# lucas-carmo/RAFT-testStuff

Hardware: AMD Instinct MI355X
Metric: sea-state cases/sec (converged RAO+PSD) (higher is better)
Workload: dtype f64; 1 GPU; C2: VolturnUS-S_example nw=1000, 512 JONSWAP sea states per GPU per step (step = per-heading wave tables + batched drag fixed point); nw=1000, submerged_nodes=53, nIter=4, headings=4, parallelism=case-sharded x1, clock_ramp_steps=920

## Files before the change

raft-teststuff_amd/csrc/rh_solve.hip:

```cpp
#include "rh_common.h"
#ifdef RH_VARIANTS
#include "../../tools/ubench/variants_src/rh_a0_common.h"
#endif

namespace rh {

#ifdef RH_PROF
static __device__ unsigned long long rh_prof[12];
#define PROF_T(v) const unsigned long long v = clock64()
#define PROF_ADD(i, x) if (tid == 0) atomicAdd(&rh_prof[i], (unsigned long long)(x))
#else
#define PROF_T(v)
#define PROF_ADD(i, x)
#endif

#ifdef RH_WGTIME
static __device__ unsigned long long rh_wgt[2 * 8192];
#endif

constexpr int kLT = 512;
constexpr int kLW = kLT / 64;
#ifndef RH_RING_A
#define RH_RING_A 4
#endif
#ifndef RH_RING_C
#define RH_RING_C 6
#endif
constexpr int kRingA1 = RH_RING_A;
constexpr int kRingC = RH_RING_C;
#ifndef RH_ONE_VOTE
#define RH_ONE_VOTE 0
#endif
#ifndef RH_OVERLAP
#define RH_OVERLAP 1
#endif
#ifndef RH_STATS_C
#define RH_STATS_C 1
#endif
#ifndef RH_XI_STORE
#define RH_XI_STORE 1
#endif
#define XI_STORE_MODE RH_XI_STORE
#ifndef RH_A_PAIR
#define RH_A_PAIR 1
#endif
constexpr int kAxC = 4;
#ifndef RH_JOINT_C
#define RH_JOINT_C 1
#endif
constexpr bool kJointC = RH_JOINT_C != 0;
#ifndef RH_JOINT_PARK
#define RH_JOINT_PARK 1
#endif
constexpr int kRingCJ = kRingC / 2;
static_assert(kRingC % 2 == 0, "the joint phase-C ring pairs its slots");
constexpr int kGhost = 1;
#ifndef RH_A_QUAD
#define RH_A_QUAD 1
#endif
#ifndef RH_LDS_LANE_BRANCH
#define RH_LDS_LANE_BRANCH 0
#endif

__device__ __forceinline__ int opaque_zero() {
  int z;
  asm volatile("s_mov_b32 %0, 0" : "=s"(z));
  return z;
}

__device__ __forceinline__ int lane_here() {
  int r;
  asm volatile("v_mbcnt_lo_u32_b32 %0, -1, 0\n\tv_mbcnt_hi_u32_b32 %0, -1, %0" : "=v"(r));
  return r;
}

template <int CTRL>
__device__ __forceinline__ double dpp_mov(double v) {
  const int lo = __builtin_amdgcn_mov_dpp(__double2loint(v), CTRL, 0xF, 0xF, true);
  const int hi = __builtin_amdgcn_mov_dpp(__double2hiint(v), CTRL, 0xF, 0xF, true);
  return __hiloint2double(hi, lo);
}

__device__ __forceinline__ double xsum32(double t) {
  const int lo = __double2loint(t), hi = __double2hiint(t);
  const auto a = __builtin_amdgcn_permlane32_swap(lo, lo, false, false);
  const auto b = __builtin_amdgcn_permlane32_swap(hi, hi, false, false);
  return __hiloint2double(b[0], a[0]) + __hiloint2double(b[1], a[1]);
}
__device__ __forceinline__ double xsum16(double t) {
  const int lo = __double2loint(t), hi = __double2hiint(t);
  const auto a = __builtin_amdgcn_permlane16_swap(lo, lo, false, false);
  const auto b = __builtin_amdgcn_permlane16_swap(hi, hi, false, false);
  return __hiloint2double(b[0], a[0]) + __hiloint2double(b[1], a[1]);
}

__device__ __forceinline__ double tbfly16(double (&u)[16], int lane) {
  const int i = lane & 15;
  const bool f0 = ((i ^ (i >> 2)) & 1) != 0, f1 = (((i >> 1) ^ (i >> 2)) & 1) != 0;
  const bool f2 = (((i >> 2) ^ (i >> 3)) & 1) != 0, f3 = ((i >> 3) & 1) != 0;
#pragma unroll
  for (int p = 0; p < 8; ++p) {
    const double keep = f0 ? u[p + 8] : u[p], send = f0 ? u[p] : u[p + 8];
    u[p] = keep + dpp_mov<0xB1>(send);
  }
#pragma unroll
  for (int p = 0; p < 4; ++p) {
    const double keep = f1 ? u[p + 4] : u[p], send = f1 ? u[p] : u[p + 4];
    u[p] = keep + dpp_mov<0x4E>(send);
  }
#pragma unroll
  for (int p = 0; p < 2; ++p) {
    const double keep = f2 ? u[p + 2] : u[p], send = f2 ? u[p] : u[p + 2];
    u[p] = keep + dpp_mov<0x141>(send);
  }
  {
    const double keep = f3 ? u[1] : u[0], send = f3 ? u[0] : u[1];
    u[0] = keep + dpp_mov<0x140>(send);
  }
  return xsum32(xsum16(u[0]));
}
__device__ __forceinline__ int tbfly16_index(int lane) {
  const int i = lane & 15;
  return 8 * ((i ^ (i >> 2)) & 1) + 4 * (((i >> 1) ^ (i >> 2)) & 1) + 2 * (((i >> 2) ^ (i >> 3)) & 1) + ((i >> 3) & 1);
}

__device__ __forceinline__ double tbfly3(double a, double b, double c, int lane) {
  const bool f0 = (lane & 1) != 0, f1 = (lane & 2) != 0;
  const double k0 = f0 ? c : a, s0 = f0 ? a : c;
  const double k1 = f0 ? 0.0 : b, s1 = f0 ? b : 0.0;
  const double u0 = k0 + dpp_mov<0xB1>(s0);
  const double u1 = k1 + dpp_mov<0xB1>(s1);
  double t = (f1 ? u1 : u0) + dpp_mov<0x4E>(f1 ? u0 : u1);
  t += dpp_mov<0x124>(t);
  t += dpp_mov<0x128>(t);
  return xsum32(xsum16(t));
}
__device__ __forceinline__ int tbfly3_index(int lane) { return 2 * (lane & 1) + ((lane >> 1) & 1); }

struct Bfly4 {
  bool f0, f1, f2;
  int vi;
  int vi8;
};
__device__ __forceinline__ Bfly4 bfly4_lane(int lane) {
  const int i = lane & 15;
  Bfly4 b;
  b.f0 = ((i ^ (i >> 2)) & 1) != 0;
  b.f1 = (((i >> 1) ^ (i >> 2)) & 1) != 0;
  b.f2 = (((i >> 2) ^ (i >> 3)) & 1) != 0;
  b.vi = lane >= 4 ? -1 : 2 * (lane & 1) + ((lane >> 1) & 1);
  b.vi8 = lane >= 8 ? -1 : 4 * b.f0 + 2 * b.f1 + b.f2;
  return b;
}
__device__ __forceinline__ double tbfly8(const double (&u)[8], const Bfly4& L) {
  const bool f0 = L.f0, f1 = L.f1, f2 = L.f2;
  double v[4], w[2];
#pragma unroll
  for (int p = 0; p < 4; ++p) v[p] = (f0 ? u[p + 4] : u[p]) + dpp_mov<0xB1>(f0 ? u[p] : u[p + 4]);
#pragma unroll
  for (int p = 0; p < 2; ++p) w[p] = (f1 ? v[p + 2] : v[p]) + dpp_mov<0x4E>(f1 ? v[p] : v[p + 2]);
  double t = (f2 ? w[1] : w[0]) + dpp_mov<0x141>(f2 ? w[0] : w[1]);
  t += dpp_mov<0x140>(t);
  return xsum32(xsum16(t));
}
__device__ __forceinline__ double tbfly4(double a, double b, double c, double d, const Bfly4& L) {
  const bool f0 = L.f0, f1 = L.f1;
  const double v0 = (f0 ? c : a) + dpp_mov<0xB1>(f0 ? a : c);
  const double v1 = (f0 ? d : b) + dpp_mov<0xB1>(f0 ? b : d);
  double t = (f1 ? v1 : v0) + dpp_mov<0x4E>(f1 ? v0 : v1);
  t += dpp_mov<0x141>(t);
  t += dpp_mov<0x140>(t);
  return xsum32(xsum16(t));
}

template <int CTRL, int ROWS>
__device__ __forceinline__ double dpp_mov_rows(double v) {
  const int lo = __builtin_amdgcn_update_dpp(0, __double2loint(v), CTRL, ROWS, 0xF, false);
  const int hi = __builtin_amdgcn_update_dpp(0, __double2hiint(v), CTRL, ROWS, 0xF, false);
  return __hiloint2double(hi, lo);
}

__device__ __forceinline__ double wave_sum63(double v) {
  v += dpp_mov<0xB1>(v);
  v += dpp_mov<0x4E>(v);
  v += dpp_mov<0x141>(v);
  v += dpp_mov<0x140>(v);
  v += dpp_mov_rows<0x142, 0xA>(v);
  v += dpp_mov_rows<0x143, 0xC>(v);
  return v;
}

__device__ __forceinline__ double t3to6_block(const double* Bm, double rx, double ry, double rz, int blk, int r, int c) {
  const double H[3][3] = {{0, rz, -ry}, {-rz, 0, rx}, {ry, -rx, 0}};
  double hc[3], hr[3];
#pragma unroll
  for (int k = 0; k < 3; ++k) {
    hc[k] = c == 0 ? H[k][0] : c == 1 ? H[k][1] : H[k][2];
    hr[k] = r == 0 ? H[0][k] : r == 1 ? H[1][k] : H[2][k];
  }
  double hcc[3];
#pragma unroll
  for (int k = 0; k < 3; ++k) hcc[k] = c == 0 ? H[0][k] : c == 1 ? H[1][k] : H[2][k];
  const double b0 = Bm[3 * r + c];
  const double b1 = Bm[3 * r + 0] * hc[0] + Bm[3 * r + 1] * hc[1] + Bm[3 * r + 2] * hc[2];
  double b2 = 0;
#pragma unroll
  for (int k = 0; k < 3; ++k) {
    const double HB = hr[0] * Bm[0 * 3 + k] + hr[1] * Bm[1 * 3 + k] + hr[2] * Bm[2 * 3 + k];
    b2 += HB * hcc[k];
  }
  return blk == 0 ? b0 : blk == 1 ? b1 : b2;
}

__host__ __device__ inline size_t solve_lds_smem(int nn, int nm, int NB, int LT = kLT, bool ser = false, int NP = 1) {
  const int LW = LT / 64;
  return sizeof(double) * ((size_t)(NP == 1 ? 12 * LT * NB : 0)
                           + (size_t)(ser && nn * 3 * LW < 27 ? 27 : nn * 3 * LW)
                           + (ser ? (size_t)0 : (size_t)nn * 36)
                           + (size_t)nn * 9
                           + (size_t)(nn + kGhost) * 6
                           + (size_t)(nn + kGhost)
                           + (size_t)nm * 18
                           + (size_t)2 * LT * NB * NP
                           + 36 + 108 + LW * 6 + 36
                           + LW)
         + sizeof(int) * ((size_t)nm + 6);
}

template <int NB, int LT = kLT, bool SER = false, int NP = 1>
__global__ __launch_bounds__(LT, LT >= 256 ? 512 / LT : 2) void k_solve_lds(CaseArgs a) {
  constexpr bool JC = kJointC && NB == 2 && LT == kLT && !SER && NP == 1;
  constexpr int LW = LT / 64;
  extern __shared__ __attribute__((aligned(16))) double smem[];
  const int tid = threadIdx.x, lane = tid & 63, wv = tid >> 6;
  const int wv_s = __builtin_amdgcn_readfirstlane(wv);
  PROF_T(tp0);
#ifdef RH_WGTIME
  const unsigned long long wgt0 = __builtin_amdgcn_s_memrealtime();
#endif
  const int slot = xcd_remap(blockIdx.x, a.c.ncase);
  const int ic = a.c.order ? a.c.order[slot] : slot;
#ifdef RH_VARIANTS
  const bool resume = a.resume != 0;
  const int stop_iter = a.stop_iter;
  if (resume && a.o.status[ic] != kCaseStopped) return;
#else
  constexpr bool resume = false;
  constexpr int stop_iter = 1 << 30;
#endif
  const rh_design& d = a.designs[a.c.design[ic]].d;
  const int nw = d.nw, nn = d.nn, nm = d.nm;
  const unsigned nw16 = (unsigned)nw * 16u;
  const double* __restrict__ node = d.node;
  const int head = a.c.head[ic];
  const size_t c6 = (size_t)ic * 6 * nw;
  const Buf bK = mkbuf(d.kproj + (size_t)head * nn * 3 * nw, (unsigned)nn * 3u * nw16);
  const Buf bFe = mkbuf(d.finer + (size_t)head * 6 * nw, 6u * nw16);
  const bool has_fx = a.c.fext != nullptr;
  const Buf bFx = mkbuf(has_fx ? a.c.fext + c6 : nullptr, has_fx ? 6u * nw16 : 0u);

  constexpr int NWP = LT * NB;
  constexpr int NBT = NB * NP;
  constexpr bool GX = NP > 1;
  constexpr int kRingA = GX ? 3 : kRingA1;
  constexpr bool kStatsC = RH_STATS_C && (XI_STORE_MODE == 1) && !SER && NB > 1;
#if RH_OVERLAP && !defined(RH_VARIANTS)
  constexpr bool kOv = !GX;
#else
  constexpr bool kOv = false;
#endif
  auto wave_maxes = [&](const double* m) {
    double mx = m[0];
    for (int w = 1; w < LW; ++w) mx = fmax(mx, m[w]);
    return mx;
  };
  cd* xl = reinterpret_cast<cd*>(smem);
  rh_c128* XL = a.o.Xi_last + c6;
  double* mbf = smem + (GX ? 0 : 12 * NWP);
  double* al = mbf + 18 * nm;
  double* red = al + 6 * (nn + kGhost);
  double* bm = red + (SER && nn * 3 * LW < 27 ? 27 : nn * 3 * LW);
  double* bd = bm + nn * 9;
  double* mbc = bd + 36;
  double* sred = mbc + 108;
  double* bsum = sred + LW * 6;
  double* bdn = bsum + 36;
  double* nt = bdn + (SER ? 0 : 36 * nn);
  double* lw = nt + nn + kGhost;
  double* lz = lw + NP * NWP;
  double* mred = lz + NP * NWP;
  int* mstart = reinterpret_cast<int*>(mred + LW);
  int* ax = reinterpret_cast<int*>(al);
  auto ax_node = [&](int k) { return k < nn ? __builtin_amdgcn_readfirstlane(ax[12 * k + 11]) : -1; };
  int* sflag = mstart + nm + 1;
  load_mbc(d, mbc, tid);
  for (int n = tid; n < nn; n += LT) {
    nt[n] = node[RH_NF_T * nn + n];
    const double aq = node[RH_NF_AQ * nn + n], cdq = node[RH_NF_CDQ * nn + n];
    const double ae = node[RH_NF_AEND * nn + n], cde = node[RH_NF_CDEND * nn + n];
    ax[12 * n + 10] = (a.all_axial || aq * cdq != 0.0 || ae * cde != 0.0) ? 1 : 0;
  }
  for (int e = tid; e < 18 * nm; e += LT) mbf[e] = d.memb[(e % 18) * nm + e / 18];
  for (int e = tid; e <= nm; e += LT) mstart[e] = e < nm ? d.mstart[e] : INT_MAX;
  for (int e = tid; e < 6 * kGhost; e += LT) al[6 * nn + e] = 0.0;
  for (int e = tid; e < kGhost; e += LT) nt[nn + e] = 0.0;
  if (tid < 5) sflag[tid] = 0;
  const int it0 = resume ? stop_iter : a.c.first_iter;
#ifdef RH_VARIANTS
  bool skip_a = a.a0 != 0 && it0 == 0;
#else
  constexpr bool skip_a = false;
#endif
  if (skip_a) {
#ifdef RH_VARIANTS
    const double* a0s = a0_block(a, ic, nw);
    const int nch = a0_chunks(nw);
    for (int e = tid; e < nn * 3; e += LT) {
      double s = 0;
      for (int ch = 0; ch < nch; ++ch) s += a0s[(size_t)ch * 3 * nn + e];
      red[e * LW] = s;
#pragma unroll
      for (int w = 1; w < LW; ++w) red[e * LW + w] = 0.0;
    }
    __syncthreads();
#endif
  }

  auto voff = [&](int b) { return (unsigned)(b < nw ? b : nw - 1) * 16u; };
  {
    const int spec = a.c.spectrum[ic];
    const double Hs = a.c.Hs[ic], Tp = a.c.Tp[ic], gam = a.c.gamma[ic];
    const rh_c128* XI0 = resume ? a.o.Xi_last + c6 : a.c.Xi_init ? a.c.Xi_init + c6 : nullptr;
#pragma unroll
    for (int j = 0; j < NBT; ++j) {
      const int b = tid + LT * j;
      const bool okb = b < nw;
      lw[b] = d.w[okb ? b : nw - 1];
#pragma unroll
      for (int c = 0; c < 6; ++c) {
        const cd x0 = okb ? (XI0 ? ld(XI0 + c * nw + b) : mk(a.c.XiStart, 0.0)) : mk(0.0, 0.0);
        if constexpr (GX) {
          if (okb && !resume) st(XL + c * nw + b, x0);
        } else {
          xl[c * NWP + b] = x0;
        }
      }
    }
#pragma unroll
    for (int j = 0; j < NBT; ++j) {
      const int b = tid + LT * j;
      const bool okb = b < nw;
      const double zz = sea_amplitude(spec, Hs, Tp, gam, lw[b], d.dw);
      lz[b] = okb ? zz : 0.0;
      if (okb && a.o.zeta) a.o.zeta[(size_t)ic * nw + b] = zz;
    }
  }
  rh_c128* Xo = a.o.Xi ? a.o.Xi + c6 : nullptr;
  rh_c128* XP = a.o.Xi_prev ? a.o.Xi_prev + c6 : nullptr;
  const double rho = d.rho;
  const int nloop = a.c.nIter + 1;
  const double tol = a.c.tol;
  int status = RH_CASE_NOT_CONVERGED, iters = nloop;
  double margin = resume && a.o.margin ? a.o.margin[ic] : INFINITY;
  const int itend = resume || stop_iter >= nloop ? nloop : stop_iter;
  __syncthreads();
  for (int n = tid; n < nn; n += LT) {
    int rank = 0, nq = 0;
    for (int k = 0; k < nn; ++k) {
      const int f = ax[12 * k + 10] & 1;
      nq += f;
      rank += k < n ? f : 0;
    }
    if (ax[12 * n + 10] & 1) ax[12 * rank + 11] = n;
    if (n >= nq) ax[12 * n + 11] = -1;
  }
  __syncthreads();
  __syncthreads();
  PROF_T(tp1);
  PROF_ADD(0, tp1 - tp0);

  auto excite = [&](int bj, cd (&F)[6]) {
    const unsigned vj = voff(bj);
    const bool okj = bj < nw;
    cd fe[6];
#pragma unroll
    for (int c = 0; c < 6; ++c) fe[c] = bld(bFe, vj, c * nw16);
#pragma unroll
    for (int c = 0; c < 6; ++c) F[c] = mk(0, 0);
    {
      cd SQ = mk(0, 0), S1 = mk(0, 0), S2 = mk(0, 0), T1 = mk(0, 0), T2 = mk(0, 0);
      auto load1 = [&](cd (&K)[2], int n) {
        const unsigned so = (unsigned)(n < nn ? n : nn - 1) * 3u * nw16;
#if RH_ABL_C_NOLOAD
        if (n >= kRingC) return;
#endif
#pragma unroll
        for (int p = 0; p < 2; ++p) K[p] = bld(bK, vj, so + (unsigned)(p + 1) * nw16);
      };
      auto load_axial = [&](cd& Kq, int k) {
        const int n = ax_node(k);
        if (n >= 0) Kq = bld(bK, vj, (unsigned)n * 3u * nw16);
        else Kq = mk(0.0, 0.0);
      };
      int m = 0, mnext = nn > 0 ? mstart[1] : 0;
      auto fold = [&]() {
#pragma unroll
        for (int i = 0; i < 6; ++i) {
          const double c1 = mbf[18 * m + RH_MF_C10 + i], c2 = mbf[18 * m + RH_MF_C20 + i];
          F[i] = add(F[i], add(scl(S1, c1), scl(S2, c2)));
        }
#pragma unroll
        for (int i = 0; i < 3; ++i) {
          const double p1 = mbf[18 * m + RH_MF_C10 + i], p2 = mbf[18 * m + RH_MF_C20 + i];
          F[3 + i] = add(F[3 + i], sub(scl(T1, p2), scl(T2, p1)));
        }
        S1 = S2 = T1 = T2 = mk(0, 0);
      };
      cd KQ[kAxC];
#pragma unroll
      for (int r = 0; r < kAxC; ++r) load_axial(KQ[r], nn > 0 ? r : nn);
      __builtin_amdgcn_sched_barrier(0);
      cd K[kRingC][2];
#pragma unroll
      for (int r = 0; r < kRingC; ++r) {
        load1(K[r], r);
        __builtin_amdgcn_sched_barrier(0);
      }
      double A1 = al[1], A2 = al[2], A3 = al[3], A4 = al[4];
      auto step = [&](cd (&K)[2], int n) {
        while (n == mnext) {
          fold();
          ++m;
          mnext = mstart[m + 1];
        }
        const double a1 = A1, a2 = A2, a3 = A3, a4 = A4;
        {
          const double* A = al + 6 * (n + 1 < nn ? n + 1 : nn);
          A1 = A[1]; A2 = A[2]; A3 = A[3]; A4 = A[4];
        }
#if RH_ABL_C_NOCOMP
        S1 = add(S1, K[0]); S2 = add(S2, K[1]);
        load1(K, n + kRingC);
        return;
#endif
        S1 = add(S1, scl(K[0], a1));
        S2 = add(S2, scl(K[1], a2));
        T1 = add(T1, scl(K[0], a3));
        T2 = add(T2, scl(K[1], a4));
        __builtin_amdgcn_sched_barrier(0);
        load1(K, n + kRingC);
        __builtin_amdgcn_sched_barrier(0);
      };
#pragma unroll 1
      for (int n = 0; n < nn; n += kRingC) {
#pragma unroll
        for (int r = 0; r < kRingC; ++r) step(K[r], n + r);
      }
      if (nn > 0) fold();
      {
        int ma = 0, mq = -1;
        auto flush = [&]() {
#pragma unroll
          for (int i = 0; i < 6; ++i) F[i] = add(F[i], scl(SQ, mbf[18 * mq + RH_MF_CQ0 + i]));
          SQ = mk(0, 0);
        };
        for (int k0 = 0; k0 < nn; k0 += kAxC) {
          if (ax_node(k0) < 0) break;
#pragma unroll
          for (int r = 0; r < kAxC; ++r) {
            const int n = ax_node(k0 + r);
            if (n >= 0) {
              while (n >= __builtin_amdgcn_readfirstlane(mstart[ma + 1])) ++ma;
              if (ma != mq) {
                if (mq >= 0) flush();
                mq = ma;
              }
              SQ = add(SQ, scl(KQ[r], al[6 * n]));
              load_axial(KQ[r], k0 + r + kAxC);
            }
          }
        }
        if (mq >= 0) flush();
      }
    }
    const double z = lz[bj];
#pragma unroll
    for (int c = 0; c < 6; ++c) F[c] = add(scl(fe[c], z), scl(F[c], z));
    if (has_fx) {
      cd fx[6];
#pragma unroll
      for (int c = 0; c < 6; ++c) fx[c] = bld(bFx, vj, c * nw16);
#pragma unroll
      for (int c = 0; c < 6; ++c) F[c] = add(F[c], mk(okj ? fx[c].r : 0.0, okj ? fx[c].i : 0.0));
    }
  };
  auto excite2 = [&](cd (&F)[2][6]) {
    unsigned vj[2];
#pragma unroll
    for (int j = 0; j < 2; ++j) vj[j] = voff(tid + LT * j);
    cd fe[2][6];
#pragma unroll
    for (int j = 0; j < 2; ++j)
#pragma unroll
      for (int c = 0; c < 6; ++c) F[j][c] = mk(0, 0);
    {
      cd SQ[2], S1[2], S2[2], T1[2], T2[2];
#pragma unroll
      for (int j = 0; j < 2; ++j) SQ[j] = S1[j] = S2[j] = T1[j] = T2[j] = mk(0, 0);
      auto load1 = [&](cd (&K)[2], int n, int j) {
        const unsigned so = (unsigned)(n < nn ? n : nn - 1) * 3u * nw16;
#pragma unroll
        for (int p = 0; p < 2; ++p) K[p] = bld(bK, vj[j], so + (unsigned)(p + 1) * nw16);
      };
      auto load_axial = [&](cd (&Kq)[2], int k) {
        const int n = ax_node(k);
        if (n >= 0) {
#pragma unroll
          for (int j = 0; j < 2; ++j) Kq[j] = bld(bK, vj[j], (unsigned)n * 3u * nw16);
        } else {
          Kq[0] = Kq[1] = mk(0.0, 0.0);
        }
      };
      int m = 0, mnext = nn > 0 ? mstart[1] : 0;
      auto fold = [&]() {
#pragma unroll
        for (int i = 0; i < 6; ++i) {
          const double c1 = mbf[18 * m + RH_MF_C10 + i], c2 = mbf[18 * m + RH_MF_C20 + i];
#pragma unroll
          for (int j = 0; j < 2; ++j) F[j][i] = add(F[j][i], add(scl(S1[j], c1), scl(S2[j], c2)));
        }
#pragma unroll
        for (int i = 0; i < 3; ++i) {
          const double p1 = mbf[18 * m + RH_MF_C10 + i], p2 = mbf[18 * m + RH_MF_C20 + i];
#pragma unroll
          for (int j = 0; j < 2; ++j) F[j][3 + i] = add(F[j][3 + i], sub(scl(T1[j], p2), scl(T2[j], p1)));
        }
#pragma unroll
        for (int j = 0; j < 2; ++j) S1[j] = S2[j] = T1[j] = T2[j] = mk(0, 0);
      };
      cd KQ[kAxC][2];
#pragma unroll
      for (int r = 0; r < kAxC; ++r) load_axial(KQ[r], nn > 0 ? r : nn);
      __builtin_amdgcn_sched_barrier(0);
      cd K[kRingCJ][2][2];
#pragma unroll
      for (int r = 0; r < kRingCJ; ++r) {
#pragma unroll
        for (int j = 0; j < 2; ++j) {
          load1(K[r][j], r, j);
          __builtin_amdgcn_sched_barrier(0);
        }
      }
      double A1 = al[1], A2 = al[2], A3 = al[3], A4 = al[4];
      auto step = [&](cd (&K)[2][2], int n) {
        while (n == mnext) {
          fold();
          ++m;
          mnext = mstart[m + 1];
        }
        const double a1 = A1, a2 = A2, a3 = A3, a4 = A4;
        {
          const double* A = al + 6 * (n + 1 < nn ? n + 1 : nn);
          A1 = A[1]; A2 = A[2]; A3 = A[3]; A4 = A[4];
        }
#pragma unroll
        for (int j = 0; j < 2; ++j) {
          S1[j] = add(S1[j], scl(K[j][0], a1));
          S2[j] = add(S2[j], scl(K[j][1], a2));
          T1[j] = add(T1[j], scl(K[j][0], a3));
          T2[j] = add(T2[j], scl(K[j][1], a4));
          __builtin_amdgcn_sched_barrier(0);
          load1(K[j], n + kRingCJ, j);
          __builtin_amdgcn_sched_barrier(0);
        }
      };
#pragma unroll 1
      for (int n = 0; n < nn; n += kRingCJ) {
#pragma unroll
        for (int r = 0; r < kRingCJ; ++r) step(K[r], n + r);
      }
      if (nn > 0) fold();
#pragma unroll
      for (int j = 0; j < 2; ++j)
#pragma unroll
        for (int c = 0; c < 6; ++c) fe[j][c] = bld(bFe, vj[j], c * nw16);
      {
        int ma = 0, mq = -1;
        auto flush = [&]() {
#pragma unroll
          for (int i = 0; i < 6; ++i) {
            const double cq = mbf[18 * mq + RH_MF_CQ0 + i];
#pragma unroll
            for (int j = 0; j < 2; ++j) F[j][i] = add(F[j][i], scl(SQ[j], cq));
          }
          SQ[0] = SQ[1] = mk(0, 0);
        };
        for (int k0 = 0; k0 < nn; k0 += kAxC) {
          if (ax_node(k0) < 0) break;
#pragma unroll
          for (int r = 0; r < kAxC; ++r) {
            const int n = ax_node(k0 + r);
            if (n >= 0) {
              while (n >= __builtin_amdgcn_readfirstlane(mstart[ma + 1])) ++ma;
              if (ma != mq) {
                if (mq >= 0) flush();
                mq = ma;
              }
              const double aq = al[6 * n];
#pragma unroll
              for (int j = 0; j < 2; ++j) SQ[j] = add(SQ[j], scl(KQ[r][j], aq));
              load_axial(KQ[r], k0 + r + kAxC);
            }
          }
        }
        if (mq >= 0) flush();
      }
    }
#pragma unroll
    for (int j = 0; j < 2; ++j) {
      const double z = lz[tid + LT * j];
#pragma unroll
      for (int c = 0; c < 6; ++c) F[j][c] = add(scl(fe[j][c], z), scl(F[j][c], z));
    }
    if (has_fx) {
#pragma unroll
      for (int j = 0; j < 2; ++j) {
        const bool okj = tid + LT * j < nw;
        cd fx[6];
#pragma unroll
        for (int c = 0; c < 6; ++c) fx[c] = bld(bFx, vj[j], c * nw16);
#pragma unroll
        for (int c = 0; c < 6; ++c) F[j][c] = add(F[j][c], mk(okj ? fx[c].r : 0.0, okj ? fx[c].i : 0.0));
      }
    }
  };

  const double hdw = 0.5 / d.dw;
  for (int it = it0; it < itend; ++it) {
    PROF_T(ta0);
    PROF_ADD(7, 1);
#pragma unroll 1
    for (int p = 0; p < NP; ++p) {
      const int pb = tid + NWP * p;
      unsigned vb[NB];
      double bz[NB];
#pragma unroll
      for (int j = 0; j < NB; ++j) {
        vb[j] = voff(pb + LT * j);
        bz[j] = lz[pb + LT * j];
      }
      cd XR[GX ? NB : 1][6];
      if constexpr (GX) {
#pragma unroll
        for (int j = 0; j < NB; ++j) {
          const int b = pb + LT * j, bc = b < nw ? b : nw - 1;
#pragma unroll
          for (int c = 0; c < 6; ++c) {
            const cd v = ld(XL + c * nw + bc);
            XR[j][c] = b < nw ? v : mk(0.0, 0.0);
          }
        }
      }
      cd B1[NB], B2[NB], E1[NB], E2[NB];
#pragma unroll
      for (int j = 0; j < NB; ++j) B1[j] = B2[j] = E1[j] = E2[j] = mk(0.0, 0.0);
      auto bin_xi = [&](int j, cd (&X)[6]) {
#pragma unroll
        for (int c = 0; c < 6; ++c) {
          if constexpr (GX) X[c] = XR[j][c];
          else X[c] = xl[c * NWP + pb + LT * j];
        }
      };
      auto member_terms = [&](int m) {
        double c1[6], c2[6];
#pragma unroll
        for (int i = 0; i < 6; ++i) {
          c1[i] = mbf[18 * m + RH_MF_C10 + i];
          c2[i] = mbf[18 * m + RH_MF_C20 + i];
        }
#pragma unroll
        for (int j = 0; j < NB; ++j) {
          cd X[6];
          bin_xi(j, X);
          cd A1 = mk(0, 0), A2 = mk(0, 0);
#pragma unroll
          for (int c = 0; c < 6; ++c) {
            A1 = add(A1, scl(X[c], c1[c]));
            A2 = add(A2, scl(X[c], c2[c]));
          }
          const cd D1 = add(add(scl(X[3], c2[0]), scl(X[4], c2[1])), scl(X[5], c2[2]));
          const cd D2 = add(add(scl(X[3], c1[0]), scl(X[4], c1[1])), scl(X[5], c1[2]));
          const double w = lw[pb + LT * j];
          B1[j] = iw(w, A1);
          B2[j] = iw(w, A2);
          E1[j] = iw(w, D1);
          E2[j] = iw(-w, D2);
        }
      };
      auto axial_term = [&](int m, cd (&Bq)[NB]) {
        double cq[6];
#pragma unroll
        for (int i = 0; i < 6; ++i) cq[i] = mbf[18 * m + RH_MF_CQ0 + i];
#pragma unroll
        for (int j = 0; j < NB; ++j) {
          cd X[6];
          bin_xi(j, X);
          cd Aq = mk(0, 0);
#pragma unroll
          for (int c = 0; c < 6; ++c) Aq = add(Aq, scl(X[c], cq[c]));
          Bq[j] = iw(lw[pb + LT * j], Aq);
        }
      };
      auto load_node = [&](cd (&K)[2][NB], int n) {
        const unsigned so = (unsigned)(n < nn ? n : nn - 1) * 3u * nw16;
#if RH_ABL_A_NOLOAD
        if (n >= kRingA) return;
#endif
#pragma unroll
        for (int j = 0; j < NB; ++j)
#pragma unroll
          for (int p = 0; p < 2; ++p) K[p][j] = bld(bK, vb[j], so + (unsigned)(p + 1) * nw16);
      };
      auto load_axial = [&](cd (&K)[NB], int k) {
        const int n = ax_node(k);
        if (n >= 0) {
          const unsigned so = (unsigned)n * 3u * nw16;
#pragma unroll
          for (int j = 0; j < NB; ++j) K[j] = bld(bK, vb[j], so);
        } else {
#pragma unroll
          for (int j = 0; j < NB; ++j) K[j] = mk(0.0, 0.0);
        }
      };
      auto node_sums = [&](const cd (&K)[2][NB], double t, double& s1, double& s2) {
        s1 = s2 = 0;
#if RH_ABL_A_NOCOMP
#pragma unroll
        for (int j = 0; j < NB; ++j) { s1 += K[0][j].r + K[0][j].i; s2 += K[1][j].r + K[1][j].i; }
        return;
#endif
#pragma unroll
        for (int j = 0; j < NB; ++j) {
          const double z = bz[j];
          const cd sp1 = sub(scl(K[0][j], z), add(B1[j], scl(E1[j], t)));
          const cd sp2 = sub(scl(K[1][j], z), add(B2[j], scl(E2[j], t)));
          s1 += abs2(sp1);
          s2 += abs2(sp2);
        }
      };
      constexpr bool kPair = RH_A_PAIR && (kRingA % 2 == 0);
      constexpr int kAx = kPair ? 4 : 3;
      const int nA = skip_a ? 0 : nn;
      cd KQ[kAx][NB];
#pragma unroll
      for (int r = 0; r < kAx; ++r) load_axial(KQ[r], nA > 0 ? r : nn);
      cd K[kRingA][2][NB];
#pragma unroll
      for (int r = 0; r < kRingA; ++r) {
        load_node(K[r], r);
        __builtin_amdgcn_sched_barrier(0);
      }
      int m = -1, mnext = 0;
      double h1 = 0.0, h2 = 0.0;
      constexpr bool kQuad = RH_A_QUAD && kPair && kRingA == 4;
      [[maybe_unused]] double u8[8] = {0.0, 0.0, 0.0, 0.0, 0.0, 0.0, 0.0, 0.0};
      const Bfly4 bl = bfly4_lane(kPair ? lane_here() : 0);
      double tn = nt[0];
#pragma unroll 1
      for (int n = 0; n < nA; n += kRingA) {
#pragma unroll
        for (int r = 0; r < kRingA; ++r) {
          const int nr = n + r;
          if (nr == mnext) {
            do { ++m; mnext = mstart[m + 1]; } while (mnext == nr);
            member_terms(m);
          }
          double s1, s2;
          node_sums(K[r], tn, s1, s2);
          asm volatile("" : "+v"(s1), "+v"(s2));
          tn = nt[nr + 1 < nn ? nr + 1 : nn];
          load_node(K[r], nr + kRingA);
          __builtin_amdgcn_sched_barrier(0);
          if constexpr (kQuad) {
            u8[2 * r] = s1;
            u8[2 * r + 1] = s2;
            if (r == kRingA - 1) {
              const double tot = tbfly8(u8, bl);
              if (bl.vi8 >= 0 && n + (bl.vi8 >> 1) < nA) {
                double& rr = red[((n + (bl.vi8 >> 1)) * 3 + 1 + (bl.vi8 & 1)) * LW + wv_s];
                rr = (GX && p > 0) ? rr + tot : tot;
              }
            }
          } else if constexpr (kPair) {
            if ((r & 1) == 0) {
              h1 = s1; h2 = s2;
            } else {
              const double tot = tbfly4(h1, h2, s1, s2, bl);
              if (bl.vi >= 0 && nr - 1 + (bl.vi >> 1) < nA) {
                double& rr = red[((nr - 1 + (bl.vi >> 1)) * 3 + 1 + (bl.vi & 1)) * LW + wv_s];
                rr = (GX && p > 0) ? rr + tot : tot;
              }
            }
          } else {
            const int ln = lane_here();
#if RH_ABL_A_NOBFLY
            const double tot = s1 + s2;
#else
            const double tot = tbfly3(s1, s2, 0.0, ln);
#endif
            if (ln < 3 && tbfly3_index(ln) < 2 && nr < nA) {
              double& rr = red[(nr * 3 + 1 + tbfly3_index(ln)) * LW + wv_s];
              rr = (GX && p > 0) ? rr + tot : tot;
            }
          }
        }
      }
      int ma = 0;
      for (int k0 = 0; k0 < nA; k0 += kAx) {
        if (ax_node(k0) < 0) break;
        double q[4] = {0.0, 0.0, 0.0, 0.0};
#pragma unroll
        for (int r = 0; r < kAx; ++r) {
          const int n = ax_node(k0 + r);
          if (n >= 0) {
            while (n >= __builtin_amdgcn_readfirstlane(mstart[ma + 1])) ++ma;
            cd Bq[NB];
            axial_term(ma, Bq);
            double s0 = 0;
#pragma unroll
            for (int j = 0; j < NB; ++j) {
              const cd sq = sub(scl(KQ[r][j], bz[j]), Bq[j]);
              s0 += abs2(sq);
            }
            q[r] = s0;
            load_axial(KQ[r], k0 + r + kAx);
          }
        }
        int vi;
        double tot;
        if constexpr (kPair) {
          tot = tbfly4(q[0], q[1], q[2], q[3], bl);
          vi = bl.vi;
        } else {
          const int ln = lane_here();
          tot = tbfly3(q[0], q[1], q[2], ln);
          vi = ln < 3 ? tbfly3_index(ln) : -1;
        }
        if (vi >= 0 && k0 + vi < nn) {
          const int n = ax[12 * (k0 + vi) + 11];
          if (n >= 0) {
            double& rr = red[n * 3 * LW + wv_s];
            rr = (GX && p > 0) ? rr + tot : tot;
          }
        }
      }
    }
#ifdef RH_VARIANTS
    skip_a = false;
#endif
    __syncthreads();
    if constexpr (kOv) {
      if (it > it0) {
        const int fl = sflag[(it - 1) & 1];
        if (a.o.margin && tid == 0) margin = closer_call(margin, wave_maxes(mred) - tol);
        if (fl & 6) {
          status = (fl & 2) ? RH_CASE_NAN : RH_CASE_SINGULAR;
          iters = it;
          break;
        }
      }
    }
    PROF_T(ta1);
    PROF_ADD(1, ta1 - ta0);
    for (int n = tid; n < nn; n += LT) {
      double fv[RH_NF_CIRC - RH_NF_XX + 2];
#pragma unroll
      for (int f = RH_NF_XX; f <= RH_NF_CIRC; ++f) fv[f - RH_NF_XX] = node[(size_t)f * nn + n];
      fv[RH_NF_CIRC - RH_NF_XX + 1] = node[(size_t)RH_NF_T * nn + n];
      __builtin_amdgcn_sched_barrier(0);
      auto F = [&](int f) { return f == RH_NF_T ? fv[RH_NF_CIRC - RH_NF_XX + 1] : fv[f - RH_NF_XX]; };
      double r3[3];
#pragma unroll
      for (int c = 0; c < 3; ++c) {
        const double* R = red + (size_t)(n * 3 + c) * LW;
        double s = 0;
#pragma unroll
        for (int w = 0; w < LW; ++w) s += R[w];
        r3[c] = s;
      }
      if (!(ax[12 * n + 10] & 1)) r3[0] = 0.0;
      auto n2 = [&](int f) { const double a = F(f), b = F(f + 1), c = F(f + 2); return a * a + b * b + c * c; };
      const double qq = n2(RH_NF_QX), pp1 = n2(RH_NF_P1X), pp2 = n2(RH_NF_P2X);
      const bool circ = F(RH_NF_CIRC) != 0.0;
      const double sums[3] = {r3[0] * qq, circ ? r3[1] * pp1 + r3[2] * pp2 : r3[1] * pp1, r3[2] * pp2};
      double B4[4];
      node_bmat_f(F, rho, sums, bm + 9 * n, B4);
      const double t = F(RH_NF_T);
      double* A = al + 6 * n;
      A[0] = B4[0] + B4[3];
      A[1] = B4[1];
      A[2] = B4[2];
      A[3] = t * B4[1];
      A[4] = t * B4[2];
      if (!SER) {
        const double rx = F(RH_NF_XX), ry = F(RH_NF_XY), rz = F(RH_NF_XZ);
#pragma unroll
        for (int e = 0; e < 36; ++e) bdn[e * nn + n] = t3to6(bm + 9 * n, rx, ry, rz, e / 6, e % 6);
      }
    }
    __syncthreads();
    if (SER) {
      const int cn = (nn * 3 * LW) / 27 > 0 ? (nn * 3 * LW) / 27 : 1;
      double se = 0.0;
      for (int n0 = 0; n0 < nn; n0 += cn) {
        const int cnt = nn - n0 < cn ? nn - n0 : cn;
        for (int nl = tid; nl < cnt; nl += LT) {
          const int n = n0 + nl;
          const double rx = nf(node, nn, RH_NF_XX, n), ry = nf(node, nn, RH_NF_XY, n), rz = nf(node, nn, RH_NF_XZ, n);
          double Bn[9];
#pragma unroll
          for (int k = 0; k < 9; ++k) Bn[k] = bm[9 * n + k];
#pragma unroll
          for (int e = 0; e < 27; ++e) red[27 * nl + e] = t3to6_block(Bn, rx, ry, rz, e / 9, (e % 9) / 3, e % 3);
        }
        __syncthreads();
        if (tid < 27)
          for (int k = 0; k < cnt; ++k) se += red[27 * k + tid];
        __syncthreads();
      }
      if (tid < 27) {
        const int blk = tid / 9, r = (tid % 9) / 3, c = tid % 3;
        if (blk == 0) bd[6 * r + c] = se;
        else if (blk == 1) bd[6 * r + 3 + c] = bd[6 * (3 + c) + r] = se;
        else bd[6 * (3 + r) + 3 + c] = se;
      }
      __syncthreads();
      if (tid < 36) bsum[tid] = mbc[36 + tid] + bd[tid];
    } else if (tid < 36) {
      double s = 0;
      const double* P = bdn + tid * nn;
      for (int n = 0; n < nn; ++n) s += P[n];
      bd[tid] = s;
      bsum[tid] = mbc[36 + tid] + s;
    }
    __syncthreads();
    PROF_T(ta2);
    PROF_ADD(2, ta2 - ta0 - (ta1 - ta0));
#ifdef RH_PROF
    unsigned long long tc_exc = 0, tc_sol = 0, tc_z = 0, tc_lu = 0;
#endif
    bool my_ok = true, my_nan = false, my_sing = false;
    double tN = 0.0, tD = 1.0;
    const bool last_it = __builtin_amdgcn_readfirstlane(it + 1 == nloop ? 1 : 0) != 0;
    auto may_be_final = [&]() -> bool {
      if (last_it) return true;
      if (__builtin_amdgcn_ballot_w64(!my_ok)) {
        if (lane == 0) __hip_atomic_store(&sflag[2], it + 1, __ATOMIC_RELAXED, __HIP_MEMORY_SCOPE_WORKGROUP);
        return false;
      }
      return __builtin_amdgcn_readfirstlane(__hip_atomic_load(&sflag[2], __ATOMIC_RELAXED, __HIP_MEMORY_SCOPE_WORKGROUP)) != it + 1;
    };
    if constexpr (kStatsC)
      if (lane < 6) sred[wv * 6 + lane] = 0.0;
    if constexpr (kOv) {
      if (tid == 0) {
        sflag[(it + 1) & 1] = 0;
        sflag[3 + ((it + 1) & 1)] = 0;
      }
    }
#if !RH_JOINT_PARK
    cd FR[6];
#pragma unroll
    for (int c = 0; c < 6; ++c) FR[c] = mk(0.0, 0.0);
#endif
#pragma unroll 1
    for (int j = 0; j < NBT; ++j) {
      const int bj = tid + LT * j;
      const bool okj = bj < nw;
      PROF_T(tc0);
      cd F[6];
      if constexpr (JC) {
        rh_c128* PK = (Xo ? Xo : a.o.Xi_last ? a.o.Xi_last + c6 : a.o.F_wave + c6) + bj;
        if (j == 0) {
          cd F2[2][6];
          excite2(F2);
#pragma unroll
          for (int c = 0; c < 6; ++c) F[c] = F2[0][c];
#if RH_JOINT_PARK
          if (bj + LT < nw) {
#pragma unroll
            for (int c = 0; c < 6; ++c) st(PK + LT + c * nw, F2[1][c]);
          }
#else
#pragma unroll
          for (int c = 0; c < 6; ++c) FR[c] = F2[1][c];
#endif
        } else {
#if RH_JOINT_PARK
#pragma unroll
          for (int c = 0; c < 6; ++c) F[c] = mk(0.0, 0.0);
          if (okj) {
#pragma unroll
            for (int c = 0; c < 6; ++c) F[c] = ld(PK + c * nw);
          }
#else
#pragma unroll
          for (int c = 0; c < 6; ++c) F[c] = FR[c];
#endif
        }
      } else {
        excite(bj, F);
      }
      if (a.o.F_wave && may_be_final()) {
        if (okj) {
#pragma unroll
          for (int c = 0; c < 6; ++c) st_nt(a.o.F_wave + c6 + c * nw + bj, F[c]);
        }
      }
      PROF_T(tc1);
#ifdef RH_PROF
      tc_exc += tc1 - tc0;
#endif
#if RH_LDS_LANE_BRANCH
      if (!okj) continue;
#else
      if (!__builtin_amdgcn_ballot_w64(okj)) continue;
#endif
      const int b = bj;
      const double w = lw[b];
      cd Z[6][6];
      {
        const int zo = opaque_zero();
        const double* zm = mbc + zo;
        const double* zb = bd + zo;
        const double* zs = bsum + zo;
        const double w2 = -(w * w);
        if (d.mb_per_bin) {
          const int bc = okj ? b : nw - 1;
          const double* M = d.M + (size_t)bc * 36;
          const double* B = d.B + (size_t)bc * 36;
#pragma unroll
          for (int r = 0; r < 6; ++r) {
#pragma unroll
            for (int c = 0; c < 6; ++c) Z[r][c] = mk(w2 * M[6 * r + c] + zm[72 + 6 * r + c], w * (B[6 * r + c] + zb[6 * r + c]));
            __builtin_amdgcn_sched_barrier(0);
          }
        } else {
#pragma unroll
          for (int r = 0; r < 6; ++r) {
#pragma unroll
            for (int c = 0; c < 6; ++c)
              Z[r][c] = mk(w2 * zm[6 * r + c] + zm[72 + 6 * r + c], w * zs[6 * r + c]);
            __builtin_amdgcn_sched_barrier(0);
          }
        }
      }
#ifdef RH_PROF
      const unsigned long long tcz = clock64();
      tc_z += tcz - tc1;
#endif
      const bool ok_lu = lu_solve<6>(Z, F);
      my_sing |= okj && !ok_lu;
#ifdef RH_PROF
      tc_lu += clock64() - tcz;
#endif
#pragma unroll
      for (int c = 0; c < 6; ++c) {
        const cd x = F[c];
        cd xlast;
        if constexpr (GX) {
          const cd v = ld(XL + c * nw + (okj ? b : nw - 1));
          xlast = okj ? v : mk(0.0, 0.0);
        } else {
          xlast = xl[c * NWP + b];
        }
        my_nan |= okj && ((x.r != x.r) || (x.i != x.i));
        const double n2 = abs2(sub(x, xlast)), den = sqrt(abs2(x)) + tol, d2 = den * den;
        const double td = tol * den;
        my_ok = my_ok && (!okj || n2 < td * td);
        const bool gt = okj && n2 * tD > tN * d2;
        tN = gt ? n2 : tN;
        tD = gt ? d2 : tD;
        [[maybe_unused]] const bool pass = n2 < td * td;
#if RH_XI_STORE == 0
        if (okj && (GX || Xo) && (pass || last_it)) st_nt(Xo + c * nw + b, x);
#elif RH_XI_STORE == 2
        if (okj && (GX || Xo) && last_it) st_nt(Xo + c * nw + b, x);
#endif
        if (okj && XP) st(XP + c * nw + b, xlast);
        const cd xr = add(scl(xlast, 0.2), scl(x, 0.8));
        if constexpr (GX) {
          if (okj) st(XL + c * nw + b, xr);
        } else {
          xl[c * NWP + b] = xr;
        }
      }
#if RH_XI_STORE == 1
      if ((GX || Xo) && may_be_final()) {
        if constexpr (kStatsC) {
          const double z = lz[b];
          const double rz = fabs(z) > 1e-6 ? 1.0 / z : 0.0;
          double m2v[6];
#pragma unroll
          for (int c = 0; c < 6; ++c) m2v[c] = okj ? abs2(c >= 3 ? scl(F[c], kRad2Deg) : F[c]) : 0.0;
          if (okj) {
#pragma unroll
            for (int c = 0; c < 6; ++c) {
              st_nt(Xo + c * nw + b, F[c]);
              if (a.o.psd) __builtin_nontemporal_store(m2v[c] * hdw, a.o.psd + ((size_t)ic * 6 + c) * nw + b);
              if (a.o.rao) st_nt(a.o.rao + ((size_t)ic * 6 + c) * nw + b, scl(F[c], rz));
            }
          }
          if (a.o.std) {
            const int ln = lane_here();
            const double t0 = tbfly3(m2v[0], m2v[1], m2v[2], ln), t1 = tbfly3(m2v[3], m2v[4], m2v[5], ln);
            if (ln < 3) {
              const int k = tbfly3_index(ln);
              sred[wv * 6 + k] += t0;
              sred[wv * 6 + 3 + k] += t1;
            }
          }
        } else if (okj) {
#pragma unroll
          for (int c = 0; c < 6; ++c) st_nt(Xo + c * nw + b, F[c]);
        }
      }
#endif
#ifdef RH_PROF
      tc_sol += clock64() - tc1;
#endif
    }
    PROF_ADD(3, tc_exc);
    PROF_ADD(4, tc_sol);
    PROF_ADD(8, tc_z);
    PROF_ADD(9, tc_lu);
    PROF_T(ta3);
    if (a.o.margin) {
      const double my_tmax = sqrt(tN) / sqrt(tD);
      const double mw = wave_max(my_tmax);
      if (lane == 0) mred[wv] = mw;
    }
    if constexpr (kOv) {
      const bool last = it + 1 == nloop;
      const unsigned long long bn = __builtin_amdgcn_ballot_w64(!my_ok), bx = __builtin_amdgcn_ballot_w64(my_nan),
                               bs = __builtin_amdgcn_ballot_w64(my_sing);
      const int bits = (bn ? 1 : 0) | (bx ? 2 : 0) | (bs ? 4 : 0);
      if (lane == 0) {
        if (bits) __hip_atomic_fetch_or(&sflag[it & 1], bits, __ATOMIC_RELAXED, __HIP_MEMORY_SCOPE_WORKGROUP);
        if (bn) __hip_atomic_store(&sflag[2], it + 1, __ATOMIC_RELAXED, __HIP_MEMORY_SCOPE_WORKGROUP);
        __hip_atomic_fetch_add(&sflag[3 + (it & 1)], 1, __ATOMIC_RELEASE, __HIP_MEMORY_SCOPE_WORKGROUP);
      }
      bool go_on = !last && bn != 0;
      if (!go_on) {
#pragma unroll 1
        while (true) {
          const int dn = __builtin_amdgcn_readfirstlane(
              __hip_atomic_load(&sflag[3 + (it & 1)], __ATOMIC_ACQUIRE, __HIP_MEMORY_SCOPE_WORKGROUP));
          const int mk = __builtin_amdgcn_readfirstlane(
              __hip_atomic_load(&sflag[2], __ATOMIC_RELAXED, __HIP_MEMORY_SCOPE_WORKGROUP));
          if (!last && mk == it + 1) {
            go_on = true;
            break;
          }
          if (dn == LW) break;
          __builtin_amdgcn_s_sleep(1);
        }
      }
      PROF_T(ta4);
      PROF_ADD(5, ta4 - ta3);
      if (go_on) continue;
      const int fl = __builtin_amdgcn_readfirstlane(
          __hip_atomic_load(&sflag[it & 1], __ATOMIC_ACQUIRE, __HIP_MEMORY_SCOPE_WORKGROUP));
      if (a.o.margin && tid == 0) margin = closer_call(margin, wave_maxes(mred) - tol);
      status = (fl & 2) ? RH_CASE_NAN : (fl & 4) ? RH_CASE_SINGULAR : (fl & 1) ? RH_CASE_NOT_CONVERGED : RH_CASE_CONVERGED;
      iters = it + 1;
      break;
    } else {
#if RH_ONE_VOTE
    {
      const unsigned long long bn = __builtin_amdgcn_ballot_w64(!my_ok), bx = __builtin_amdgcn_ballot_w64(my_nan),
                               bs = __builtin_amdgcn_ballot_w64(my_sing);
      const int bits = (bn ? 1 : 0) | (bx ? 2 : 0) | (bs ? 4 : 0);
      if (lane == 0 && bits) atomicOr(&sflag[it & 1], bits);
    }
    __syncthreads();
    const int fl = sflag[it & 1];
    if (tid == 0) sflag[(it + 1) & 1] = 0;
    const int all_ok = !(fl & 1), any_nan = fl & 2, any_sing = fl & 4;
    if (a.o.margin && tid == 0) {
      double mx = mred[0];
      for (int w = 1; w < LW; ++w) mx = fmax(mx, mred[w]);
      margin = closer_call(margin, mx - tol);
    }
#else
    const int all_ok = __syncthreads_and(my_ok ? 1 : 0);
    if (a.o.margin && tid == 0) {
      double mx = mred[0];
      for (int w = 1; w < LW; ++w) mx = fmax(mx, mred[w]);
      margin = closer_call(margin, mx - tol);
    }
    const int any_nan = __syncthreads_or(my_nan ? 1 : 0);
    const int any_sing = __syncthreads_or(my_sing ? 1 : 0);
#endif
    PROF_T(ta4);
    PROF_ADD(5, ta4 - ta3);
    if (any_nan) {
      status = RH_CASE_NAN;
      iters = it + 1;
      break;
    }
    if (any_sing) {
      status = RH_CASE_SINGULAR;
      iters = it + 1;
      break;
    }
    if (all_ok) {
      status = RH_CASE_CONVERGED;
      iters = it + 1;
      break;
    }
    }
  }

  if (status == RH_CASE_NOT_CONVERGED && itend < nloop) {
#pragma unroll 1
    for (int j = 0; j < NB && !GX; ++j) {
      const int b = tid + LT * j;
      if (b >= nw) continue;
#pragma unroll 1
      for (int c = 0; c < 6; ++c) st(a.o.Xi_last + c6 + c * nw + b, xl[c * NWP + b]);
    }
    if (tid == 0) {
      a.o.status[ic] = kCaseStopped;
      if (a.o.margin) a.o.margin[ic] = margin;
    }
    return;
  }

#ifdef RH_WGTIME
  if (tid == 0 && blockIdx.x < 8192) {
    rh_wgt[2 * blockIdx.x] = wgt0;
    rh_wgt[2 * blockIdx.x + 1] = __builtin_amdgcn_s_memrealtime();
  }
#endif
  PROF_T(te0);
  if (tid == 0) {
    a.o.iters[ic] = iters;
    a.o.status[ic] = status;
    if (a.o.margin) a.o.margin[ic] = margin;
  }
  if (a.o.B_drag && tid < 36) a.o.B_drag[(size_t)ic * 36 + tid] = bd[tid];
  if (a.o.Bmat)
    for (int e = tid; e < nn * 9; e += LT) a.o.Bmat[(size_t)ic * a.bmat_nn * 9 + e] = bm[e];
  if (a.o.Z) {
#pragma unroll 1
    for (int j = 0; j < NBT; ++j) {
      const int b = tid + LT * j;
      if (b >= nw) continue;
      const double w = lw[b], w2 = -(w * w);
      rh_c128* Zo = a.o.Z + ((size_t)ic * nw + b) * 36;
#pragma unroll 1
      for (int e = 0; e < 36; ++e) {
        const double M = d.mb_per_bin ? d.M[(size_t)b * 36 + e] : mbc[e];
        const double B = d.mb_per_bin ? d.B[(size_t)b * 36 + e] : mbc[36 + e];
        st(Zo + e, mk(w2 * M + mbc[72 + e], w * (B + bd[e])));
      }
    }
  }
  const bool failed = status == RH_CASE_NAN || status == RH_CASE_SINGULAR;
  if (failed && a.o.F_wave) {
#pragma unroll 1
    for (int j = 0; j < NBT; ++j) {
      const int b = tid + LT * j;
      if (b >= nw) continue;
#pragma unroll
      for (int c = 0; c < 6; ++c) st(a.o.F_wave + ((size_t)ic * 6 + c) * nw + b, mk(NAN, NAN));
    }
  }
  double ss[6] = {0, 0, 0, 0, 0, 0};
  if (!kStatsC || failed) {
#pragma unroll
  for (int j = 0; j < NBT; ++j) {
    const int b = tid + LT * j;
    if (b >= nw || !Xo) continue;
    const double z = lz[b];
    const double rz = fabs(z) > 1e-6 ? 1.0 / z : 0.0;
#pragma unroll
    for (int c = 0; c < 6; ++c) {
      cd x;
      if (failed) {
        x = mk(NAN, NAN);
        st(Xo + c * nw + b, x);
      } else {
        x = ld(Xo + c * nw + b);
      }
      const cd xd = c >= 3 ? scl(x, kRad2Deg) : x;
      const double m2 = abs2(xd);
      ss[c] += m2;
      if (a.o.psd) a.o.psd[((size_t)ic * 6 + c) * nw + b] = m2 * hdw;
      if (a.o.rao) st(a.o.rao + ((size_t)ic * 6 + c) * nw + b, failed ? x : scl(x, rz));
    }
  }
  }
  if (a.o.std) {
    if (!kStatsC || failed) {
#pragma unroll
      for (int c = 0; c < 6; ++c) {
        const double s = wave_sum(ss[c]);
        if (lane == 0) sred[wv * 6 + c] = s;
      }
    }
    __syncthreads();
    if (tid < 6) {
      double s = 0;
      for (int w = 0; w < LW; ++w) s += sred[w * 6 + tid];
      a.o.std[(size_t)ic * 6 + tid] = sqrt(0.5 * s);
    }
  }
  PROF_T(te1);
  PROF_ADD(6, te1 - te0);
}

}
```

raft-teststuff_amd/csrc/rh_solve_split.hip:

```cpp
#define RH_JOINT_C 0
#define k_solve_lds k_solve_lds_split
#include "rh_solve.hip"
#undef k_solve_lds
#include "rh_solve_launch.h"

namespace rh {

hipError_t launch_solve_split(dim3 grid, dim3 block, size_t lsm, hipStream_t s, const CaseArgs& a) {
  hipLaunchKernelGGL((k_solve_lds_split<2>), grid, block, lsm, s, a);
  return hipGetLastError();
}

hipError_t occupancy_solve_split(int* per_cu, int threads, size_t lsm) {
  return hipOccupancyMaxActiveBlocksPerMultiprocessor(per_cu, k_solve_lds_split<2>, threads, lsm);
}

}
```

Measured before the change: 952,700 cases/s.

## Batch LDS loads in drag-matrix build and replace axial-node ranking with ballot scan

```diff
diff --git a/raft-teststuff_amd/csrc/rh_solve.hip b/raft-teststuff_amd/csrc/rh_solve.hip
--- a/raft-teststuff_amd/csrc/rh_solve.hip
+++ b/raft-teststuff_amd/csrc/rh_solve.hip
@@ -49,6 +49,9 @@
 #define RH_JOINT_C 1
 #endif
 constexpr bool kJointC = RH_JOINT_C != 0;
+#ifndef RH_BATCH_B
+#define RH_BATCH_B 1
+#endif
 #ifndef RH_JOINT_PARK
 #define RH_JOINT_PARK 1
 #endif
@@ -61,6 +64,8 @@
 #ifndef RH_LDS_LANE_BRANCH
 #define RH_LDS_LANE_BRANCH 0
 #endif
+
+__device__ __forceinline__ double abs2_re(cd a) { return __builtin_fma(a.r, a.r, a.i * a.i); }
 
 __device__ __forceinline__ int opaque_zero() {
   int z;
@@ -212,6 +217,29 @@
   return blk == 0 ? b0 : blk == 1 ? b1 : b2;
 }
 
+__device__ __forceinline__ double t3to6_fma(const double (&B)[9], double rx, double ry, double rz, int i, int j) {
+  auto fma = [](double a, double b, double c) { return __builtin_fma(a, b, c); };
+  auto bh = [&](int a, int c) {
+    const double b0 = B[3 * a], b1 = B[3 * a + 1], b2 = B[3 * a + 2];
+    return c == 0 ? fma(b2, ry, fma(b0, 0.0, -(b1 * rz)))
+         : c == 1 ? fma(b2, -rx, fma(b0, rz, b1 * 0.0))
+                  : fma(b2, 0.0, fma(b1, rx, -(b0 * ry)));
+  };
+  auto hb = [&](int a, int k, bool alt) {
+    const double b0 = B[k], b1 = B[3 + k], b2 = B[6 + k];
+    return a == 0 ? fma(-ry, b2, fma(0.0, b0, b1 * rz))
+         : a == 1 ? fma(rx, b2, fma(0.0, b1, -(b0 * rz)))
+                  : fma(0.0, b2, alt ? fma(-b1, rx, b0 * ry) : fma(b0, ry, -(b1 * rx)));
+  };
+  if (i < 3 && j < 3) return B[3 * i + j];
+  if (i < 3) return bh(i, j - 3);
+  if (j < 3) return bh(j, i - 3);
+  const int a = i - 3, c = j - 3;
+  const double h0 = c == 0 ? 0.0 : c == 1 ? -rz : ry, h1 = c == 0 ? rz : c == 1 ? 0.0 : -rx;
+  const double h2 = c == 0 ? -ry : c == 1 ? rx : 0.0;
+  return fma(hb(a, 2, false), h2, fma(hb(a, 1, a == 2 && c < 2), h1, fma(hb(a, 0, false), h0, 0.0)));
+}
+
 __host__ __device__ inline size_t solve_lds_smem(int nn, int nm, int NB, int LT = kLT, bool ser = false, int NP = 1) {
   const int LW = LT / 64;
   return sizeof(double) * ((size_t)(NP == 1 ? 12 * LT * NB : 0)
@@ -231,6 +259,8 @@
 __global__ __launch_bounds__(LT, LT >= 256 ? 512 / LT : 2) void k_solve_lds(CaseArgs a) {
   constexpr bool JC = kJointC && NB == 2 && LT == kLT && !SER && NP == 1;
   constexpr int LW = LT / 64;
+  constexpr bool kBatchS = RH_BATCH_B != 0 && !SER;
+  constexpr int kSumB = 16;
   extern __shared__ __attribute__((aligned(16))) double smem[];
   const int tid = threadIdx.x, lane = tid & 63, wv = tid >> 6;
   const int wv_s = __builtin_amdgcn_readfirstlane(wv);
@@ -294,11 +324,21 @@
   auto ax_node = [&](int k) { return k < nn ? __builtin_amdgcn_readfirstlane(ax[12 * k + 11]) : -1; };
   int* sflag = mstart + nm + 1;
   load_mbc(d, mbc, tid);
-  for (int n = tid; n < nn; n += LT) {
-    nt[n] = node[RH_NF_T * nn + n];
-    const double aq = node[RH_NF_AQ * nn + n], cdq = node[RH_NF_CDQ * nn + n];
-    const double ae = node[RH_NF_AEND * nn + n], cde = node[RH_NF_CDEND * nn + n];
-    ax[12 * n + 10] = (a.all_axial || aq * cdq != 0.0 || ae * cde != 0.0) ? 1 : 0;
+  for (int n = tid; n < nn; n += LT) nt[n] = node[RH_NF_T * nn + n];
+  if (wv_s == 0) {
+    int nq = 0;
+    for (int n0 = 0; n0 < nn; n0 += 64) {
+      const int n = n0 + lane, nc = n < nn ? n : nn - 1;
+      const double aq = node[RH_NF_AQ * nn + nc], cdq = node[RH_NF_CDQ * nn + nc];
+      const double ae = node[RH_NF_AEND * nn + nc], cde = node[RH_NF_CDEND * nn + nc];
+      const bool f = n < nn && (a.all_axial || aq * cdq != 0.0 || ae * cde != 0.0);
+      const unsigned long long mask = __ballot(f);
+      const int below = __builtin_amdgcn_mbcnt_hi((unsigned)(mask >> 32), __builtin_amdgcn_mbcnt_lo((unsigned)mask, 0u));
+      if (n < nn) ax[12 * n + 10] = f ? 1 : 0;
+      if (f) ax[12 * (nq + below) + 11] = n;
+      nq += __popcll(mask);
+    }
+    for (int k = nq + lane; k < nn; k += 64) ax[12 * k + 11] = -1;
   }
   for (int e = tid; e < 18 * nm; e += LT) mbf[e] = d.memb[(e % 18) * nm + e / 18];
   for (int e = tid; e <= nm; e += LT) mstart[e] = e < nm ? d.mstart[e] : INT_MAX;
@@ -363,18 +403,6 @@
   int status = RH_CASE_NOT_CONVERGED, iters = nloop;
   double margin = resume && a.o.margin ? a.o.margin[ic] : INFINITY;
   const int itend = resume || stop_iter >= nloop ? nloop : stop_iter;
-  __syncthreads();
-  for (int n = tid; n < nn; n += LT) {
-    int rank = 0, nq = 0;
-    for (int k = 0; k < nn; ++k) {
-      const int f = ax[12 * k + 10] & 1;
-      nq += f;
-      rank += k < n ? f : 0;
-    }
-    if (ax[12 * n + 10] & 1) ax[12 * rank + 11] = n;
-    if (n >= nq) ax[12 * n + 11] = -1;
-  }
-  __syncthreads();
   __syncthreads();
   PROF_T(tp1);
   PROF_ADD(0, tp1 - tp0);
@@ -872,7 +900,8 @@
     }
     PROF_T(ta1);
     PROF_ADD(1, ta1 - ta0);
-    for (int n = tid; n < nn; n += LT) {
+    const int tid_b = kBatchS ? wv_s * 64 + lane_here() : tid;
+    for (int n = tid_b; n < nn; n += LT) {
       double fv[RH_NF_CIRC - RH_NF_XX + 2];
 #pragma unroll
       for (int f = RH_NF_XX; f <= RH_NF_CIRC; ++f) fv[f - RH_NF_XX] = node[(size_t)f * nn + n];
@@ -880,13 +909,29 @@
       __builtin_amdgcn_sched_barrier(0);
       auto F = [&](int f) { return f == RH_NF_T ? fv[RH_NF_CIRC - RH_NF_XX + 1] : fv[f - RH_NF_XX]; };
       double r3[3];
-#pragma unroll
-      for (int c = 0; c < 3; ++c) {
-        const double* R = red + (size_t)(n * 3 + c) * LW;
-        double s = 0;
-#pragma unroll
-        for (int w = 0; w < LW; ++w) s += R[w];
-        r3[c] = s;
+      if constexpr (kBatchS) {
+        double pr[3][LW];
+#pragma unroll
+        for (int c = 0; c < 3; ++c)
+#pragma unroll
+          for (int w = 0; w < LW; ++w) pr[c][w] = red[(size_t)(n * 3 + c) * LW + w];
+        __builtin_amdgcn_sched_barrier(0);
+#pragma unroll
+        for (int c = 0; c < 3; ++c) {
+          double s = 0;
+#pragma unroll
+          for (int w = 0; w < LW; ++w) s += pr[c][w];
+          r3[c] = s;
+        }
+      } else {
+#pragma unroll
+        for (int c = 0; c < 3; ++c) {
+          const double* R = red + (size_t)(n * 3 + c) * LW;
+          double s = 0;
+#pragma unroll
+          for (int w = 0; w < LW; ++w) s += R[w];
+          r3[c] = s;
+        }
       }
       if (!(ax[12 * n + 10] & 1)) r3[0] = 0.0;
       auto n2 = [&](int f) { const double a = F(f), b = F(f + 1), c = F(f + 2); return a * a + b * b + c * c; };
@@ -894,7 +939,14 @@
       const bool circ = F(RH_NF_CIRC) != 0.0;
       const double sums[3] = {r3[0] * qq, circ ? r3[1] * pp1 + r3[2] * pp2 : r3[1] * pp1, r3[2] * pp2};
       double B4[4];
-      node_bmat_f(F, rho, sums, bm + 9 * n, B4);
+      double Bn[9];
+      if constexpr (kBatchS) {
+        node_bmat_f(F, rho, sums, Bn, B4);
+#pragma unroll
+        for (int k = 0; k < 9; ++k) bm[9 * n + k] = Bn[k];
+      } else {
+        node_bmat_f(F, rho, sums, bm + 9 * n, B4);
+      }
       const double t = F(RH_NF_T);
       double* A = al + 6 * n;
       A[0] = B4[0] + B4[3];
@@ -905,7 +957,8 @@
       if (!SER) {
         const double rx = F(RH_NF_XX), ry = F(RH_NF_XY), rz = F(RH_NF_XZ);
 #pragma unroll
-        for (int e = 0; e < 36; ++e) bdn[e * nn + n] = t3to6(bm + 9 * n, rx, ry, rz, e / 6, e % 6);
+        for (int e = 0; e < 36; ++e)
+          bdn[e * nn + n] = kBatchS ? t3to6_fma(Bn, rx, ry, rz, e / 6, e % 6) : t3to6(bm + 9 * n, rx, ry, rz, e / 6, e % 6);
       }
     }
     __syncthreads();
@@ -938,8 +991,29 @@
       if (tid < 36) bsum[tid] = mbc[36 + tid] + bd[tid];
     } else if (tid < 36) {
       double s = 0;
-      const double* P = bdn + tid * nn;
-      for (int n = 0; n < nn; ++n) s += P[n];
+      const double* P = bdn + (kBatchS ? lane_here() : tid) * nn;
+      if constexpr (kBatchS) {
+        int n = 0;
+        for (; n + kSumB <= nn; n += kSumB) {
+          double p[kSumB];
+#pragma unroll
+          for (int k = 0; k < kSumB; ++k) p[k] = P[n + k];
+          __builtin_amdgcn_sched_barrier(0);
+#pragma unroll
+          for (int k = 0; k < kSumB; ++k) s += p[k];
+        }
+        if (n < nn) {
+          double p[kSumB - 1];
+#pragma unroll
+          for (int k = 0; k < kSumB - 1; ++k) p[k] = P[n + k];
+          __builtin_amdgcn_sched_barrier(0);
+#pragma unroll
+          for (int k = 0; k < kSumB - 1; ++k)
+            if (n + k < nn) s += p[k];
+        }
+      } else {
+        for (int n = 0; n < nn; ++n) s += P[n];
+      }
       bd[tid] = s;
       bsum[tid] = mbc[36 + tid] + s;
     }
@@ -1102,7 +1176,7 @@
           const double rz = fabs(z) > 1e-6 ? 1.0 / z : 0.0;
           double m2v[6];
 #pragma unroll
-          for (int c = 0; c < 6; ++c) m2v[c] = okj ? abs2(c >= 3 ? scl(F[c], kRad2Deg) : F[c]) : 0.0;
+          for (int c = 0; c < 6; ++c) m2v[c] = okj ? abs2_re(c >= 3 ? scl(F[c], kRad2Deg) : F[c]) : 0.0;
           if (okj) {
 #pragma unroll
             for (int c = 0; c < 6; ++c) {
diff --git a/raft-teststuff_amd/csrc/rh_solve_split.hip b/raft-teststuff_amd/csrc/rh_solve_split.hip
--- a/raft-teststuff_amd/csrc/rh_solve_split.hip
+++ b/raft-teststuff_amd/csrc/rh_solve_split.hip
@@ -1,4 +1,5 @@
 #define RH_JOINT_C 0
+#define RH_BATCH_B 0
 #define k_solve_lds k_solve_lds_split
 #include "rh_solve.hip"
 #undef k_solve_lds
```

After: 992,900 cases/s (median of 6 runs). 1.04x the previous value.
